# hyperledger-labs/bdls

Hardware: AMD Instinct MI355X
Metric: P-256 ECDSA verifies/sec (fused SHA-256, bit-exact vs Go crypto/ecdsa + Fabric low-S) (higher is better)
Workload: dtype u32; 1 GPU; BASELINE config 2: 1048576 records/GPU, 256B messages, 65536 distinct keys, 1/16 corrupted, fused SHA-256; records_per_gpu=1048576, records_total=1048576, msg_len=256, nkeys=65536, corrupt_den=16, parallelism=shard1 (no collective)

## Files before the change

### bdls_amd/csrc/ec30.h

```cpp
#pragma once
#include "fp30.h"

namespace bh {

struct J30 {
  uint32_t X[9], Y[9], Z[9];
};

BH_HD void j_copy(J30& r, const J30& p) {
  f_copy(r.X, p.X);
  f_copy(r.Y, p.Y);
  f_copy(r.Z, p.Z);
}

BH_HD void j_sel(J30& r, bool c, const J30& a, const J30& b) {
  f_sel(r.X, c, a.X, b.X);
  f_sel(r.Y, c, a.Y, b.Y);
  f_sel(r.Z, c, a.Z, b.Z);
}

template <class F>
BH_HD void j_dbl(J30& r, const J30& p) {
  if constexpr (F::a_is_minus3) {
    uint32_t delta[9], gamma[9], bt[9], t0[9], t1[9], u[9], alpha[9];
    f_sqr<F>(delta, p.Z);
    f_sqr<F>(gamma, p.Y);
    f_mul<F>(bt, p.X, gamma);
    f_sub<F, 32>(t0, p.X, delta);
    f_add(t1, p.X, delta);
    f_mul<F>(u, t0, t1);
    f_mulc<3>(alpha, u);
    f_add(t0, p.Y, p.Z);
    f_sqr<F>(t0, t0);
    f_sub2<F, 32>(r.Z, t0, gamma, delta);
    f_sqr<F>(u, alpha);
    f_mulc<8>(t0, bt);
    f_sub<F, 32>(r.X, u, t0);
    f_mulc<12>(t0, bt);
    f_sub<F, 32>(t0, t0, u);
    f_mul<F>(t0, alpha, t0);
    f_sqr<F>(gamma, gamma);
    f_mulc<8>(gamma, gamma);
    f_sub<F, 32>(r.Y, t0, gamma);
  } else {
    uint32_t A[9], B[9], Cc[9], D[9], E[9], t[9], t2[9];
    f_sqr<F>(A, p.X);
    f_sqr<F>(B, p.Y);
    f_mul<F>(t, p.Y, p.Z);
    f_sqr<F>(Cc, B);
    f_add(t2, p.X, B);
    f_sqr<F>(t2, t2);
    f_mulc<2>(r.Z, t);
    f_add(t, A, Cc);
    f_sub<F, 32>(t2, t2, t);
    f_mulc<2>(D, t2);
    f_mulc<3>(E, A);
    f_sqr<F>(t, E);
    f_mulc<3>(t2, D);
    f_sub<F, 32>(t2, t2, t);
    f_mulc<2>(D, D);
    f_reduce<F>(D, D);
    f_sub<F, 32>(r.X, t, D);
    f_mul<F>(t, E, t2);
    f_mulc<8>(Cc, Cc);
    f_sub<F, 32>(r.Y, t, Cc);
  }
}

template <class F>
BH_HD void j_dblu(J30& r, J30& pp, const J30& p) {
  if constexpr (F::a_is_minus3) {
    uint32_t delta[9], gamma[9], bt[9], t0[9], t1[9], u[9], alpha[9];
    f_sqr<F>(delta, p.Z);
    f_sqr<F>(gamma, p.Y);
    f_mul<F>(bt, p.X, gamma);
    f_sub<F, 32>(t0, p.X, delta);
    f_add(t1, p.X, delta);
    f_mul<F>(u, t0, t1);
    f_mulc<3>(alpha, u);
    f_add(t0, p.Y, p.Z);
    f_sqr<F>(t0, t0);
    f_sub2<F, 32>(r.Z, t0, gamma, delta);
    f_sqr<F>(u, alpha);
    f_mulc<8>(t0, bt);
    f_sub<F, 32>(r.X, u, t0);
    f_mulc<4>(pp.X, bt);
    f_mulc<12>(t0, bt);
    f_sub<F, 32>(t0, t0, u);
    f_mul<F>(t0, alpha, t0);
    f_sqr<F>(gamma, gamma);
    f_mulc<8>(pp.Y, gamma);
    f_sub<F, 32>(r.Y, t0, pp.Y);
    f_copy(pp.Z, r.Z);
  } else {
    uint32_t A[9], B[9], Cc[9], D[9], E[9], t[9], t2[9];
    f_sqr<F>(A, p.X);
    f_sqr<F>(B, p.Y);
    f_mul<F>(t, p.Y, p.Z);
    f_sqr<F>(Cc, B);
    f_add(t2, p.X, B);
    f_sqr<F>(t2, t2);
    f_mulc<2>(r.Z, t);
    f_add(t, A, Cc);
    f_sub<F, 32>(t2, t2, t);
    f_mulc<2>(D, t2);
    f_reduce<F>(D, D);
    f_copy(pp.X, D);
    f_mulc<3>(E, A);
    f_sqr<F>(t, E);
    f_mulc<3>(t2, D);
    f_sub<F, 32>(t2, t2, t);
    f_mulc<2>(D, D);
    f_sub<F, 32>(r.X, t, D);
    f_mul<F>(t, E, t2);
    f_mulc<8>(pp.Y, Cc);
    f_sub<F, 32>(r.Y, t, pp.Y);
    f_copy(pp.Z, r.Z);
  }
}

template <class F>
BH_HD void j_zaddu(J30& r, J30& p, const J30& q) {
  uint32_t t1[9], c[9], w1[9], w2[9], t2[9], d[9], t3[9];
  f_sub<F, 64>(t1, p.X, q.X);
  f_sqr<F>(c, t1);
  f_mul<F>(w1, p.X, c);
  f_mul<F>(w2, q.X, c);
  f_sub<F, 64>(t2, p.Y, q.Y);
  f_sqr<F>(d, t2);
  f_sub<F, 32>(t3, w1, w2);
  f_mul<F>(p.Y, p.Y, t3);
  f_sub2<F, 32>(r.X, d, w1, w2);
  f_sub<F, 64>(t3, w1, r.X);
  f_mul<F>(t3, t2, t3);
  f_sub<F, 32>(r.Y, t3, p.Y);
  f_mul<F>(r.Z, p.Z, t1);
  f_copy(p.X, w1);
  f_copy(p.Z, r.Z);
}

template <class F>
BH_HD bool j_degenerate(const uint32_t z3[9], const uint32_t rr[9], bool* same_y) {
  const bool degenerate = f_is_zero2<F>(z3);
  if (degenerate) {
    uint32_t t[9];
    f_reduce<F>(t, rr);
    uint32_t z = 0;
    for (int i = 0; i < 9; i++) z |= t[i];
    *same_y = (z == 0);
  } else {
    *same_y = false;
  }
  return degenerate;
}

template <class F, bool CO>
BH_HD bool j_add_impl(J30& r, J30* pz, const J30& p, const J30& q, bool neg, bool* same_y) {
  uint32_t z1z1[9], z2z2[9], u1[9], u2[9], s1[9], s2[9], h[9], rr[9], t[9], hh[9], hhh[9], w[9];
  f_sqr<F>(z1z1, p.Z);
  f_sqr<F>(z2z2, q.Z);
  f_mul<F>(u1, p.X, z2z2);
  f_mul<F>(u2, q.X, z1z1);
  f_mul<F>(t, q.Z, z2z2);
  f_mul<F>(s1, p.Y, t);
  f_mul<F>(t, p.Z, z1z1);
  f_mul<F>(s2, q.Y, t);
  f_sub<F, 32>(h, u2, u1);
  f_csub<F, 32>(rr, neg, s2, s1);
  f_sqr<F>(hh, h);
  f_mul<F>(hhh, hh, h);
  f_mul<F>(u1, u1, hh);
  f_sqr<F>(t, rr);
  f_add2x(w, hhh, u1);
  f_sub<F, 32>(r.X, t, w);
  f_addsub<F, 32>(u2, w, u1, t);
  f_mul<F>(u2, rr, u2);
  f_mul<F>(s1, s1, hhh);
  f_sub<F, 32>(r.Y, u2, s1);
  f_mul<F>(t, p.Z, q.Z);
  f_mul<F>(r.Z, t, h);
  if constexpr (CO) {
    f_copy(pz->X, u1);
    f_copy(pz->Y, s1);
    f_copy(pz->Z, r.Z);
  }
  return j_degenerate<F>(r.Z, rr, same_y);
}

template <class F>
BH_HD bool j_add(J30& r, const J30& p, const J30& q, bool* same_y) {
  return j_add_impl<F, false>(r, nullptr, p, q, false, same_y);
}
template <class F>
BH_HD bool j_add_co(J30& r, J30& pz, const J30& p, const J30& q, bool* same_y, bool neg = false) {
  return j_add_impl<F, true>(r, &pz, p, q, neg, same_y);
}

template <class F, bool CO>
BH_HD bool j_madd_impl(J30& r, J30* pz, const J30& p, const uint32_t x2[9], const uint32_t y2[9],
                       bool neg, bool* same_y) {
  uint32_t z1z1[9], u2[9], s2[9], h[9], rr[9], t[9], hh[9], hhh[9], v[9], w[9];
  f_sqr<F>(z1z1, p.Z);
  f_mul<F>(u2, x2, z1z1);
  f_mul<F>(t, p.Z, z1z1);
  f_mul<F>(s2, y2, t);
  f_sub<F, 64>(h, u2, p.X);
  f_csub<F, 96>(rr, neg, s2, p.Y);
  f_sqr<F>(hh, h);
  f_mul<F>(hhh, hh, h);
  f_mul<F>(v, p.X, hh);
  f_sqr<F>(t, rr);
  f_add2x(w, hhh, v);
  f_sub<F, 32>(r.X, t, w);
  f_addsub<F, 32>(s2, w, v, t);
  f_mul<F>(s2, rr, s2);
  f_mul<F>(t, p.Y, hhh);
  f_sub<F, 32>(r.Y, s2, t);
  f_mul<F>(r.Z, p.Z, h);
  if constexpr (CO) {
    f_copy(pz->X, v);
    f_copy(pz->Y, t);
    f_copy(pz->Z, r.Z);
  }
  return j_degenerate<F>(r.Z, rr, same_y);
}

template <class F>
BH_HD bool j_madd(J30& r, const J30& p, const uint32_t x2[9], const uint32_t y2[9], bool* same_y,
                  bool neg = false) {
  return j_madd_impl<F, false>(r, nullptr, p, x2, y2, neg, same_y);
}
template <class F>
BH_HD bool j_madd_co(J30& r, J30& pz, const J30& p, const uint32_t x2[9], const uint32_t y2[9],
                     bool* same_y, bool neg = false) {
  return j_madd_impl<F, true>(r, &pz, p, x2, y2, neg, same_y);
}

template <class F>
BH_HD bool j_on_curve(const uint32_t x[9], const uint32_t y[9]) {
  uint32_t l[9], rhs[9], t[9], b[9];
  f_sqr<F>(l, y);
  f_sqr<F>(t, x);
  f_mul<F>(rhs, t, x);
  if constexpr (F::a_is_minus3) {
    f_mulc<3>(t, x);
    f_sub<F, 32>(rhs, rhs, t);
  }
  f_const(b, F::b_m);
  f_add(rhs, rhs, b);
  f_reduce<F>(rhs, rhs);
  f_canon<F>(l, l);
  return f_eq(l, rhs);
}

}
```

### bdls_amd/csrc/fp30.h

```cpp
#pragma once
#include "bh_common.h"
#include "curve_consts.h"

#ifndef BH_ZFILTER
#define BH_ZFILTER 0
#endif

namespace bh {

constexpr uint32_t kM30 = 0x3fffffffu;
constexpr int kL = 9;

BH_HD void f_copy(uint32_t r[9], const uint32_t a[9]) {
#pragma unroll
  for (int i = 0; i < 9; i++) r[i] = a[i];
}

BH_HD void f_sel(uint32_t r[9], bool c, const uint32_t a[9], const uint32_t b[9]) {
#pragma unroll
  for (int i = 0; i < 9; i++) r[i] = c ? a[i] : b[i];
}

template <class C>
BH_HD void f_const(uint32_t r[9], const C& c) {
#pragma unroll
  for (int i = 0; i < 9; i++) r[i] = c[i];
}

template <uint32_t K>
BH_HD void mac_k(uint64_t& c, uint32_t m) {
#if defined(__HIP_DEVICE_COMPILE__)
  uint32_t k = K;
  asm("" : "+s"(k));
  c += (uint64_t)m * k;
#else
  c += (uint64_t)m * K;
#endif
}

template <class F>
BH_HD void f_redc(uint32_t r[9], uint64_t C[17]) {
  uint64_t acc = 0;
  if constexpr (F::sparse_p256) {
#pragma unroll
    for (int k = 0; k < 8; k++) {
      const uint32_t m = (uint32_t)C[k];
      mac_k<64u>(C[k + 3], m);
      mac_k<4096u>(C[k + 6], m);
      mac_k<F::p[7]>(C[k + 7], m);
      mac_k<F::p[8]>(C[k + 8], m);
      mac_k<4u>(C[k + 1], (uint32_t)(C[k] >> 32));
    }
#pragma unroll
    for (int k = 8; k < 17; k++) {
      acc += C[k];
      const uint32_t m = (uint32_t)acc & kM30;
      if (k == 8) {
        mac_k<64u>(C[11], m);
        mac_k<4096u>(C[14], m);
        mac_k<F::p[7]>(C[15], m);
        mac_k<F::p[8]>(C[16], m);
      } else {
        r[k - 9] = m;
      }
      acc >>= 30;
    }
  } else {
#pragma unroll
    for (int k = 0; k < 17; k++) {
      acc += C[k];
      if (k < 9) {
        const uint32_t m = ((uint32_t)acc * F::n0) & kM30;
        acc += (uint64_t)m * F::p[0];
#pragma unroll
        for (int j = 1; j < 9; j++)
          if (F::p[j]) C[k + j] += (uint64_t)m * F::p[j];
      } else {
        r[k - 9] = (uint32_t)acc & kM30;
      }
      acc >>= 30;
    }
  }
  r[8] = (uint32_t)acc;
}

template <class F>
BH_HD void f_mul(uint32_t r[9], const uint32_t a[9], const uint32_t b[9]) {
  uint64_t C[17];
#pragma unroll
  for (int k = 0; k < 17; k++) C[k] = 0;
#pragma unroll
  for (int i = 0; i < 9; i++)
#pragma unroll
    for (int j = 0; j < 9; j++) C[i + j] += (uint64_t)a[i] * b[j];
  f_redc<F>(r, C);
}

template <class F>
BH_HD void f_sqr(uint32_t r[9], const uint32_t a[9]) {
  uint64_t C[17];
  uint32_t d[9];
#pragma unroll
  for (int i = 0; i < 9; i++) d[i] = a[i] << 1;
#pragma unroll
  for (int k = 0; k < 17; k++) C[k] = 0;
#pragma unroll
  for (int i = 0; i < 9; i++) {
    C[2 * i] += (uint64_t)a[i] * a[i];
#pragma unroll
    for (int j = i + 1; j < 9; j++) C[i + j] += (uint64_t)d[i] * a[j];
  }
  f_redc<F>(r, C);
}

BH_HD void f_add(uint32_t r[9], const uint32_t a[9], const uint32_t b[9]) {
  uint32_t c = 0;
#pragma unroll
  for (int i = 0; i < 8; i++) {
    const uint32_t t = a[i] + b[i] + c;
    r[i] = t & kM30;
    c = t >> 30;
  }
  r[8] = a[8] + b[8] + c;
}

template <class F, int K>
BH_HD void f_sub(uint32_t r[9], const uint32_t a[9], const uint32_t b[9]) {
  static_assert(K == 32 || K == 64, "K");
  uint32_t c = 0;
#pragma unroll
  for (int i = 0; i < 8; i++) {
    const uint32_t kk = (K == 32) ? F::k32[i] : F::k64[i];
    const uint32_t t = a[i] + kk - b[i] + c;
    r[i] = t & kM30;
    c = t >> 30;
  }
  const uint32_t k8 = (K == 32) ? F::k32[8] : F::k64[8];
  r[8] = a[8] + k8 - b[8] + c;
}

struct Limbs9 {
  uint32_t v[9];
};
template <class F, int K, int B>
constexpr Limbs9 kp_borrowed() {
  Limbs9 r{};
  uint64_t c = 0;
  for (int i = 0; i < 9; i++) {
    const uint64_t t = (uint64_t)F::p[i] * (uint64_t)K + c;
    const uint64_t n = i < 8 ? (t & kM30) : t;
    c = i < 8 ? (t >> 30) : 0;
    r.v[i] = (uint32_t)(n + (i < 8 ? ((uint64_t)B << 30) : 0) - (i > 0 ? (uint64_t)B : 0));
  }
  return r;
}
template <class F, int K, int B>
struct KpB {
  static constexpr Limbs9 k = kp_borrowed<F, K, B>();
  static_assert(k.v[8] < (1u << 26), "K p's top limb covers the borrow");
};

BH_HD void f_add2x(uint32_t r[9], const uint32_t a[9], const uint32_t b[9]) {
  uint32_t c = 0;
#pragma unroll
  for (int i = 0; i < 8; i++) {
    const uint32_t t = a[i] + (b[i] << 1) + c;
    r[i] = t & kM30;
    c = t >> 30;
  }
  r[8] = a[8] + (b[8] << 1) + c;
}

template <class F, int K>
BH_HD void f_addsub(uint32_t r[9], const uint32_t a[9], const uint32_t b[9], const uint32_t c[9]) {
  static_assert(K == 32 || K == 64, "K");
  uint32_t cy = 0;
#pragma unroll
  for (int i = 0; i < 8; i++) {
    const uint32_t kk = (K == 32) ? F::k32[i] : F::k64[i];
    const uint32_t t = a[i] + b[i] + kk + cy - c[i];
    r[i] = t & kM30;
    cy = t >> 30;
  }
  const uint32_t k8 = (K == 32) ? F::k32[8] : F::k64[8];
  r[8] = a[8] + b[8] + k8 + cy - c[8];
}

template <class F, int K>
BH_HD void f_sub2(uint32_t r[9], const uint32_t a[9], const uint32_t b[9], const uint32_t c[9]) {
  constexpr Limbs9 kk = KpB<F, K, 2>::k;
  uint32_t cy = 0;
#pragma unroll
  for (int i = 0; i < 8; i++) {
    const uint32_t t = a[i] + kk.v[i] + cy - b[i] - c[i];
    r[i] = t & kM30;
    cy = t >> 30;
  }
  r[8] = a[8] + kk.v[8] + cy - b[8] - c[8];
}

template <class F, int K>
BH_HD void f_csub(uint32_t r[9], bool neg, const uint32_t s[9], const uint32_t y[9]) {
  constexpr Limbs9 kk = KpB<F, K, 2>::k;
  uint32_t cy = 0;
#pragma unroll
  for (int i = 0; i < 8; i++) {
    const uint32_t x = neg ? 0u - s[i] : s[i];
    const uint32_t t = kk.v[i] + x + cy - y[i];
    r[i] = t & kM30;
    cy = t >> 30;
  }
  const uint32_t x8 = neg ? 0u - s[8] : s[8];
  r[8] = kk.v[8] + x8 + cy - y[8];
}

template <class F, int K>
BH_HD void f_neg(uint32_t r[9], const uint32_t a[9]) {
  const uint32_t z[9] = {0, 0, 0, 0, 0, 0, 0, 0, 0};
  f_sub<F, K>(r, z, a);
}

template <uint32_t C>
BH_HD void f_mulc(uint32_t r[9], const uint32_t a[9]) {
  uint64_t c = 0;
#pragma unroll
  for (int i = 0; i < 8; i++) {
    const uint64_t t = (uint64_t)a[i] * C + c;
    r[i] = (uint32_t)t & kM30;
    c = t >> 30;
  }
  r[8] = a[8] * C + (uint32_t)c;
}

template <class F>
BH_HD void f_canon(uint32_t r[9], const uint32_t a[9]) {
  uint32_t d[9];
  int32_t c = 0;
#pragma unroll
  for (int i = 0; i < 8; i++) {
    const int32_t t = (int32_t)a[i] - (int32_t)F::p[i] + c;
    d[i] = (uint32_t)t & kM30;
    c = t >> 30;
  }
  const int32_t t8 = (int32_t)a[8] - (int32_t)F::p[8] + c;
  d[8] = (uint32_t)t8;
  f_sel(r, t8 >= 0, d, a);
}

template <class F>
BH_HD void f_reduce(uint32_t r[9], const uint32_t a[9]) {
  uint32_t one[9];
  f_const(one, F::r1);
  f_mul<F>(r, a, one);
  f_canon<F>(r, r);
}

BH_HD bool f_eq(const uint32_t a[9], const uint32_t b[9]) {
  uint32_t x = 0;
#pragma unroll
  for (int i = 0; i < 9; i++) x |= a[i] ^ b[i];
  return x == 0;
}

template <class F>
BH_HD bool f_is_zero2(const uint32_t a[9]) {
#if BH_ZFILTER
  if (a[0] != 0u && a[0] != F::p[0]) return false;
#endif
  uint32_t z = 0, q = 0;
#pragma unroll
  for (int i = 0; i < 9; i++) {
    z |= a[i];
    q |= a[i] ^ F::p[i];
  }
  return z == 0 || q == 0;
}

BH_HD void f_from_u256(uint32_t r[9], const uint32_t a[8]) {
  r[0] = a[0] & kM30;
#pragma unroll
  for (int i = 1; i < 8; i++) {
    const int lo = 30 * i;
    const int w = lo >> 5, s = lo & 31;
    uint32_t v = a[w] >> s;
    if (s > 2 && w + 1 < 8) v |= a[w + 1] << (32 - s);
    r[i] = v & kM30;
  }
  r[8] = a[7] >> 16;
}

BH_HD void f_to_u256(uint32_t r[8], const uint32_t a[9]) {
#pragma unroll
  for (int w = 0; w < 8; w++) {
    const int bit = 32 * w;
    const int i = bit / 30, s = bit % 30;
    uint32_t v = a[i] >> s;
    if (i + 1 < 9) v |= a[i + 1] << (30 - s);
    if (s > 28 && i + 2 < 9) v |= a[i + 2] << (60 - s);
    r[w] = v;
  }
}

template <class F>
BH_HD void f_to_mont(uint32_t r[9], const uint32_t a[9]) {
  uint32_t r2[9];
  f_const(r2, F::r2);
  f_mul<F>(r, a, r2);
}

template <class F>
BH_HD void f_sqrn(uint32_t r[9], const uint32_t a[9], int k) {
  f_copy(r, a);
#pragma unroll 1
  for (int i = 0; i < k; i++) f_sqr<F>(r, r);
}

template <class F>
BH_HD void f_sqrn_mul(uint32_t r[9], const uint32_t a[9], int k, const uint32_t b[9]) {
  f_sqrn<F>(r, a, k);
  f_mul<F>(r, r, b);
}

template <class F>
BH_HD void f_inv(uint32_t r[9], const uint32_t a[9]) {
  uint32_t e2[9], e3[9], t[9], u[9], acc[9];
  f_sqrn_mul<F>(e2, a, 1, a);
  f_sqrn_mul<F>(e3, e2, 1, a);
  if constexpr (F::sparse_p256) {
    uint32_t e15[9], e32[9];
    f_sqrn_mul<F>(t, e3, 3, e3);
    f_sqrn_mul<F>(u, t, 6, t);
    f_sqrn_mul<F>(e15, u, 3, e3);
    f_sqrn_mul<F>(t, e15, 15, e15);
    f_sqrn_mul<F>(e32, t, 2, e2);
    f_sqrn_mul<F>(acc, e32, 32, a);
    f_sqrn<F>(acc, acc, 96);
    f_sqrn_mul<F>(acc, acc, 32, e32);
    f_sqrn_mul<F>(acc, acc, 32, e32);
    f_sqrn_mul<F>(acc, acc, 30, t);
    f_sqrn_mul<F>(acc, acc, 2, a);
  } else {
    uint32_t e11[9], e22[9], e44[9];
    f_sqrn_mul<F>(t, e3, 3, e3);
    f_sqrn_mul<F>(u, t, 3, e3);
    f_sqrn_mul<F>(e11, u, 2, e2);
    f_sqrn_mul<F>(e22, e11, 11, e11);
    f_sqrn_mul<F>(e44, e22, 22, e22);
    f_sqrn_mul<F>(t, e44, 44, e44);
    f_sqrn_mul<F>(u, t, 88, t);
    f_sqrn_mul<F>(t, u, 44, e44);
    f_sqrn_mul<F>(acc, t, 3, e3);
    f_sqrn_mul<F>(acc, acc, 23, e22);
    f_sqrn_mul<F>(acc, acc, 5, a);
    f_sqrn_mul<F>(acc, acc, 3, e2);
    f_sqrn_mul<F>(acc, acc, 2, a);
  }
  f_copy(r, acc);
}

}
```

### bdls_amd/csrc/verify.h

```cpp
#pragma once
#include <type_traits>

#include "blake2b.h"
#include "der.h"
#include "fe.h"
#include "ec30.h"
#include "sha256.h"
#include "sha3.h"

namespace bh {

enum : uint32_t {
  BHF_HASH_SHA256 = 1u,
  BHF_NO_LOW_S = 2u,
  BHF_HASH_SHA3_256 = 8u,
  BHF_BDLS_PREHASHED = 0x100u,
};

enum : int { HK_GIVEN_OR_SHA256 = 0, HK_SHA3_256 = 1 };

enum : uint8_t { ST_R2OK = 0x80u };

struct BatchIn {
  const uint8_t* pub;
// ... 1223 lines not shown
template <class P, class Raw>
BH_HD void reg_window(uint32_t* tab, uint32_t win, const J30& B, Raw& raw) {
  J30 Bz, S;
  uint32_t z[9];
  raw.store(0u, B);
  f_copy(z, B.Z);
  raw.store_z(0u, z);
  j_dblu<P>(S, Bz, B);
  raw.store(1u, S);
  f_mul<P>(z, z, S.Z);
  raw.store_z(1u, z);
#pragma unroll 1
  for (uint32_t j = 2; j < (uint32_t)kKEnt; j++) {
    J30 T;
    j_zaddu<P>(T, Bz, S);
    raw.store(j, T);
    f_mul<P>(z, z, T.Z);
    raw.store_z(j, z);
    j_copy(S, T);
  }
  uint32_t inv[9];
  f_inv_sg<P>(inv, z);
#pragma unroll 1
  for (uint32_t j = (uint32_t)kKEnt; j-- > 0;) {
    J30 E;
    raw.load(E, j);
    uint32_t zi[9], x[9], y[9];
    if (j > 0) {
      uint32_t pz[9];
      raw.load_z(pz, j - 1u);
      f_mul<P>(zi, inv, pz);
      f_mul<P>(inv, inv, E.Z);
    } else {
      f_copy(zi, inv);
    }
    ll_to_affine<P>(x, y, E, zi);
    llaff_store(tab + kRegWin, win * (uint32_t)kKEnt + j, x, y);
  }
}

struct RegSlotRaw {
  uint32_t* tab;
  BH_HDM void store(uint32_t j, const J30& P) { ktab_store(tab + kRegWinRaw, 0, j, P); }
  BH_HDM void load(J30& P, uint32_t j) const { ktab_load(P, tab + kRegWinRaw, 0, j); }
  BH_HDM void store_z(uint32_t j, const uint32_t z[9]) { z_store(tab + kRegWinPre + 12u * j, z); }
  BH_HDM void load_z(uint32_t z[9], uint32_t j) const { z_load(z, tab + kRegWinPre + 12u * j); }
};

template <class P>
BH_HD void ktab_build_aff(uint32_t* tab, const Work& w, uint32_t rec) {
  J30 B;
  ld9(B.X, w.qx, rec, w.ns);
  ld9(B.Y, w.qy, rec, w.ns);
  f_const(B.Z, P::r1);
  RegSlotRaw raw{tab};
#pragma unroll 1
  for (uint32_t win = 0; win < (uint32_t)kKWin; win++) {
    reg_window<P>(tab, win, B, raw);
    if (win + 1u < (uint32_t)kKWin) {
#pragma unroll 1
      for (int d = 0; d < kKW; d++) j_dbl<P>(B, B);
    }
  }
}

template <class P>
BH_HD void reg_build(uint32_t* tab, const Work& w, uint32_t rec) {
  lltab_build<P>(tab, w, rec);
  ktab_build_aff<P>(tab, w, rec);
}
template <class P>
BH_HD void reg_build_comb(uint32_t* tab, const Work& w, uint32_t rec, uint32_t* scr = nullptr) {
  lltab_build<P>(tab, w, rec, scr);
}

template <class P>
using CvOf = typename std::conditional<P::a_is_minus3 != 0, Cv_p256, Cv_k1>::type;

BH_HD void ll_column(const uint64_t sl[kLLTeeth], int j, uint32_t& idx, bool& neg) {
  uint32_t m = 0;
#pragma unroll
  for (int t = 0; t + 1 < kLLTeeth; t++) m |= (uint32_t)((sl[t] >> j) & 1ull) << t;
  neg = ((sl[kLLTeeth - 1] >> j) & 1ull) == 0ull;
  idx = neg ? (~m & (kLLEnt - 1u)) : m;
}

template <class P>
BH_HD void ll_slices(uint64_t sl[kLLTeeth], const uint32_t u2[8]) {
  using Cv = CvOf<P>;
  const uint32_t add = (u2[0] & 1u) ? 0u : ~0u;
  uint32_t k[9], c[9];
  uint64_t cy = 0;
#pragma unroll
  for (int q = 0; q < 8; q++) {
    cy += (uint64_t)u2[q] + (Cv::n[q] & add);
    k[q] = (uint32_t)cy;
    cy >>= 32;
  }
  k[8] = (uint32_t)cy;
#pragma unroll
  for (int q = 0; q < 8; q++) c[q] = (k[q] >> 1) | (k[q + 1] << 31);
  c[8] = 0u;
  c[(kLLTS - 1) >> 5] |= 1u << ((kLLTS - 1) & 31);
#pragma unroll
  for (int t = 0; t < kLLTeeth; t++) {
    const int lo = kLLSpace * t, wd = lo >> 5, sh = lo & 31;
    uint64_t x = (uint64_t)c[wd] >> sh;
    if (wd + 1 < 9) x |= (uint64_t)c[wd + 1] << (32 - sh);
    if (wd + 2 < 9 && sh + kLLSpace > 64) x |= (uint64_t)c[wd + 2] << (64 - sh);
    sl[t] = x & ((1ull << kLLSpace) - 1ull);
  }
}

template <class P>
BH_HD void q_llcomb(J30& A, bool& a_inf, const Work& w, uint32_t i, const uint32_t* tab,
                    uint32_t stride = 0) {
  uint32_t u2[8], one[9];
  ld8(u2, w.r, i, w.ns);
  f_const(one, P::r1);
  uint64_t sl[kLLTeeth];
  ll_slices<P>(sl, u2);
  uint32_t idx;
  bool neg;
  ll_column(sl, kLLSpace - 1, idx, neg);
  if (stride) llent_load(A.X, A.Y, tab + idx * stride);
  else llaff_load(A.X, A.Y, tab, idx);
  f_copy(A.Z, one);
  a_inf = false;
#pragma unroll 1
  for (int j = kLLSpace - 2; j >= 0; j--) {
    j_dbl<P>(A, A);
    ll_column(sl, j, idx, neg);
    uint32_t tx[9], ty[9], nty[9];
    if (stride) llent_load(tx, ty, tab + idx * stride);
    else llaff_load(tx, ty, tab, idx);
    f_neg<P, 64>(nty, ty);
    f_sel(ty, neg, nty, ty);
    bool same;
    const bool deg = j_madd<P>(A, A, tx, ty, &same);
    if (a_inf || deg) {
      if (a_inf || same) {
        J30 T;
        f_copy(T.X, tx);
        f_copy(T.Y, ty);
        f_copy(T.Z, one);
        if (a_inf) j_copy(A, T);
        else j_dbl<P>(A, T);
        a_inf = false;
      } else {
        a_inf = true;
      }
    }
  }
}

#ifndef BH_GFOLD
#define BH_GFOLD 3
#endif
constexpr int kGF = BH_GFOLD;
static_assert(kGF >= 1 && kGF <= 4 && (kLLSpace - 1) % kGF == 0,
              "column groups of the folded G tables tile columns 1 .. s - 1");
constexpr int kGFBits = (kLLTeeth - 1) + (kGF - 1) * kLLTeeth;
constexpr uint32_t kG2Ent = 1u << kGFBits;
constexpr uint32_t kG1Ent = kLLEnt;
constexpr int kGAdds = (kLLSpace - 1) / kGF + 1;
constexpr uint32_t kGOdd = 1u << (kGF - 1);
constexpr uint32_t kGBase = (uint32_t)kLLTeeth * kGOdd;
constexpr size_t kG2Words = (size_t)(kG2Ent + kG1Ent + kGBase) * kLLAff;
constexpr size_t kGCombWords = (size_t)kCombWindows * kCombEntries * kGEntry;
constexpr size_t kGTabAllWords = kGCombWords + kG2Words;
static_assert(kGCombWords % 4 == 0, "folded tables 16-byte aligned");
BH_HD const uint32_t* g2_of(const uint32_t* gtab) { return gtab + kGCombWords; }

template <class P>
BH_HD void scalar_g_affine(const uint32_t v[9], uint32_t x[9], uint32_t y[9]) {
  uint32_t gx[9], gy[9];
  f_const(gx, P::gx_m);
  f_const(gy, P::gy_m);
  int topbit = 287;
  while (topbit > 0 && !((v[topbit >> 5] >> (topbit & 31)) & 1u)) topbit--;
  J30 A;
  f_copy(A.X, gx);
  f_copy(A.Y, gy);
  f_const(A.Z, P::r1);
  for (int b = topbit - 1; b >= 0; b--) {
    j_dbl<P>(A, A);
    if ((v[b >> 5] >> (b & 31)) & 1u) {
      bool same;
      (void)j_madd<P>(A, A, gx, gy, &same);
    }
  }
  uint32_t z[9], zi[9], zi2[9];
  f_reduce<P>(z, A.Z);
  f_inv<P>(zi, z);
  f_sqr<P>(zi2, zi);
  f_mul<P>(x, A.X, zi2);
  f_mul<P>(zi2, zi2, zi);
  f_mul<P>(y, A.Y, zi2);
  f_reduce<P>(x, x);
  f_reduce<P>(y, y);
}

template <class P>
BH_HD void gtab2_base(uint32_t k, uint32_t* g2) {
  const uint32_t i = k / kGOdd, m = k % kGOdd;
  uint32_t v[9] = {0, 0, 0, 0, 0, 0, 0, 0, 0};
  const int b = kLLSpace * (int)i;
  const uint64_t mag = (uint64_t)(2u * m + 1u) << (b & 31);
  v[b >> 5] = (uint32_t)mag;
  if ((b >> 5) + 1 < 9) v[(b >> 5) + 1] = (uint32_t)(mag >> 32);
  uint32_t x[9], y[9];
  scalar_g_affine<P>(v, x, y);
  llaff_store(g2, kG2Ent + kG1Ent + k, x, y);
}

template <class P>
BH_HD void gtab2_entry(uint32_t t, uint32_t* g2) {
  constexpr uint32_t top = 1u << (kLLTeeth - 1), all = (1u << kLLTeeth) - 1u;
  int c[kLLTeeth];
  for (int i = 0; i < kLLTeeth; i++) c[i] = 0;
  if (t < kG2Ent) {
    for (int cc = 0; cc < kGF; cc++) {
      const uint32_t bits = cc == kGF - 1 ? (top | (t >> ((kGF - 1) * kLLTeeth)))
                                          : (t >> (cc * kLLTeeth)) & all;
      for (int i = 0; i < kLLTeeth; i++) c[i] += (2 * (int)((bits >> i) & 1u) - 1) << cc;
    }
  } else {
    const uint32_t b = top | (t - kG2Ent);
    for (int i = 0; i < kLLTeeth; i++) c[i] = 2 * (int)((b >> i) & 1u) - 1;
  }
  J30 A;
  llaff_load(A.X, A.Y, g2, kG2Ent + kG1Ent + (uint32_t)(kLLTeeth - 1) * kGOdd +
                               (uint32_t)((c[kLLTeeth - 1] - 1) / 2));
  f_const(A.Z, P::r1);
  for (int i = kLLTeeth - 2; i >= 0; i--) {
    const int a = c[i] < 0 ? -c[i] : c[i];
    uint32_t bx[9], by[9];
    llaff_load(bx, by, g2, kG2Ent + kG1Ent + (uint32_t)i * kGOdd + (uint32_t)((a - 1) / 2));
    if (c[i] < 0) f_neg<P, 64>(by, by);
    bool same;
    (void)j_madd<P>(A, A, bx, by, &same);
  }
  uint32_t zi[9], x[9], y[9];
  f_inv_sg<P>(zi, A.Z);
  ll_to_affine<P>(x, y, A, zi);
  llaff_store(g2, t, x, y);
}

BH_HD void g2_column(const uint64_t gl[kLLTeeth], int j, uint32_t& idx, bool& neg) {
  if (j == 0) {
    ll_column(gl, 0, idx, neg);
    idx += kG2Ent;
    return;
  }
  constexpr uint32_t all = (1u << kLLTeeth) - 1u;
  uint32_t col[kGF];
#pragma unroll
  for (int cc = 0; cc < kGF; cc++) {
    uint32_t b = 0;
#pragma unroll
    for (int t = 0; t < kLLTeeth; t++) b |= (uint32_t)((gl[t] >> (j + cc)) & 1ull) << t;
    col[cc] = b;
  }
  neg = ((col[kGF - 1] >> (kLLTeeth - 1)) & 1u) == 0u;
  uint32_t x = col[kGF - 1] & (all >> 1);
  if (neg) x = ~col[kGF - 1] & (all >> 1);
#pragma unroll
  for (int cc = kGF - 2; cc >= 0; cc--) x = (x << kLLTeeth) | ((neg ? ~col[cc] : col[cc]) & all);
  idx = x;
}

template <class P>
BH_HD void ll_madd(J30& A, bool& a_inf, const uint32_t tx[9], uint32_t ty[9], bool neg,
                   const uint32_t one[9]) {
  bool same;
  const bool deg = j_madd<P>(A, A, tx, ty, &same, neg);
  if (a_inf || deg) {
    if (neg) f_neg<P, 64>(ty, ty);
    if (a_inf || same) {
      J30 T;
      f_copy(T.X, tx);
      f_copy(T.Y, ty);
      f_copy(T.Z, one);
      if (a_inf) j_copy(A, T);
      else j_dbl<P>(A, T);
      a_inf = false;
    } else {
      a_inf = true;
    }
  }
}

template <class P>
BH_HD void ll_dbladd(J30& A, bool& a_inf, const uint32_t tx[9], uint32_t ty[9], bool neg,
                     const uint32_t one[9]) {
  if (a_inf) {
    if (neg) f_neg<P, 64>(ty, ty);
    f_copy(A.X, tx);
    f_copy(A.Y, ty);
    f_copy(A.Z, one);
    a_inf = false;
    return;
  }
  J30 R, Az;
  bool same;
  if (j_madd_co<P>(R, Az, A, tx, ty, &same, neg)) {
    if (neg) f_neg<P, 64>(ty, ty);
    J30 T;
    f_copy(T.X, tx);
    f_copy(T.Y, ty);
    f_copy(T.Z, one);
    if (same) {
      j_dbl<P>(A, T);
      (void)j_madd<P>(A, A, tx, ty, &same);
    }
    return;
  }
  j_zaddu<P>(A, R, Az);
  if (f_is_zero2<P>(A.Z)) a_inf = true;
}

template <class P>
BH_HD void q_llcomb_g(J30& A, bool& a_inf, const Work& w, uint32_t i, const uint32_t* tab,
                      uint32_t stride, const uint32_t* g2) {
  uint32_t u2[8], u1[8], one[9];
  ld8(u2, w.r, i, w.ns);
  ld8(u1, w.e, i, w.ns);
  f_const(one, P::r1);
  uint64_t sl[kLLTeeth], gl[kLLTeeth];
  ll_slices<P>(sl, u2);
  ll_slices<P>(gl, u1);
  uint32_t idx;
  bool neg;
  ll_column(sl, kLLSpace - 1, idx, neg);
  if (stride) llent_load(A.X, A.Y, tab + idx * stride);
  else llaff_load(A.X, A.Y, tab, idx);
  f_copy(A.Z, one);
  a_inf = false;
  uint32_t gx[9], gy[9], gidx;
  bool gneg;
  g2_column(gl, kLLSpace - kGF, gidx, gneg);
  llaff_load(gx, gy, g2, gidx);
#pragma unroll 1
  for (int j = kLLSpace - 2; j >= 0; j--) {
    {
      uint32_t tx[9], ty[9];
      ll_column(sl, j, idx, neg);
      if (stride) llent_load(tx, ty, tab + idx * stride);
      else llaff_load(tx, ty, tab, idx);
      ll_dbladd<P>(A, a_inf, tx, ty, neg, one);
    }
    if (j == 0 || (j - 1) % kGF == 0) {
      ll_madd<P>(A, a_inf, gx, gy, gneg, one);
      if (j > 0) {
        g2_column(gl, j > kGF ? j - kGF : 0, gidx, gneg);
        llaff_load(gx, gy, g2, gidx);
      }
    }
  }
}

template <class P>
BH_HD bool stage_keycomb_fold(const Work& w, uint32_t i, const uint32_t* tab, uint32_t stride,
                              const uint32_t* g2) {
  J30 A;
  bool a_inf;
  q_llcomb_g<P>(A, a_inf, w, i, tab, stride, g2);
  return finish_check<P>(w, i, A, a_inf, A, true);
}

#ifndef BH_LADDER_CSUB
#define BH_LADDER_CSUB 1
#endif
template <class P>
BH_HD void j_dbladd(J30& A, bool& a_inf, J30& T, bool neg) {
  if (a_inf) {
    if (neg) f_neg<P, 64>(T.Y, T.Y);
    j_copy(A, T);
    a_inf = false;
    return;
  }
  J30 R, Az;
  bool same;
  if (j_add_co<P>(R, Az, A, T, &same, neg)) {
    if (neg) f_neg<P, 64>(T.Y, T.Y);
    if (same) {
      J30 D;
      j_dbl<P>(D, T);
      (void)j_add<P>(A, D, T, &same);
    }
    return;
  }
  j_zaddu<P>(A, R, Az);
  if (f_is_zero2<P>(A.Z)) a_inf = true;
}

BH_HD bool g_fold_pos(int p) { return p == 0 || (p >= 1 && p <= kLLSpace - kGF && (p - 1) % kGF == 0); }

template <class P>
BH_HD void q_ladder_odd_g(J30& A, bool& a_inf, const Work& w, uint32_t i, uint32_t wave,
                          uint32_t lane, const uint32_t* g2) {
  using Cv = CvOf<P>;
  uint32_t u2[8], u1[8], qx[9], qy[9], one[9];
  ld8(u2, w.r, i, w.ns);
  ld8(u1, w.e, i, w.ns);
  ld9(qx, w.qx, i, w.ns);
  ld9(qy, w.qy, i, w.ns);
  f_const(one, P::r1);
  {
    J30 Qa, D, S;
    f_copy(Qa.X, qx);
    f_copy(Qa.Y, qy);
    f_copy(Qa.Z, one);
    j_dblu<P>(D, S, Qa);
    qtab_store(w.qtab, wave, 0, lane, S);
#pragma unroll 1
    for (uint32_t m = 1; m < (uint32_t)kQTab; m++) {
      J30 Sn;
      j_zaddu<P>(Sn, D, S);
      qtab_store(w.qtab, wave, m, lane, Sn);
      j_copy(S, Sn);
    }
  }
  uint32_t K[9];
  {
    const uint32_t add = (u2[0] & 1u) ? 0u : ~0u;
    uint32_t k[9];
    uint64_t cy = 0;
#pragma unroll
    for (int q = 0; q < 8; q++) {
      cy += (uint64_t)u2[q] + (Cv::n[q] & add);
      k[q] = (uint32_t)cy;
      cy >>= 32;
    }
    k[8] = (uint32_t)cy;
    K[0] = k[0] << 30;
#pragma unroll
    for (int q = 1; q < 9; q++) K[q] = (k[q] << 30) | (k[q - 1] >> 2);
  }
  uint64_t gl[kLLTeeth];
  ll_slices<P>(gl, u1);
  uint32_t gx[9], gy[9], gidx;
  bool gneg;
  int gp = kLLSpace - kGF;
  g2_column(gl, gp, gidx, gneg);
  llaff_load(gx, gy, g2, gidx);
  auto g_add = [&]() {
    ll_madd<P>(A, a_inf, gx, gy, gneg, one);
    if (gp > 0) {
      gp = gp > kGF ? gp - kGF : 0;
      g2_column(gl, gp, gidx, gneg);
      llaff_load(gx, gy, g2, gidx);
    }
  };
  qtab_load(A, w.qtab, wave, (K[8] >> 30) & 1u, lane);
  a_inf = false;
#pragma unroll 1
  for (int win = 50; win >= 0; win--) {
    const uint32_t b = (K[8] >> 25) & 31u;
#pragma unroll
    for (int q = 8; q > 0; q--) K[q] = (K[q] << 5) | (K[q - 1] >> 27);
    K[0] <<= 5;
    const bool neg = b < 16u;
    const uint32_t mag = neg ? 31u - 2u * b : 2u * b - 31u;
    J30 T;
    qtab_load(T, w.qtab, wave, (mag - 1u) >> 1, lane);
#pragma unroll 1
    for (int d = 1; d <= 4; d++) {
      j_dbl<P>(A, A);
      if (g_fold_pos(5 * win + 5 - d)) g_add();
    }
#if BH_LADDER_CSUB
    j_dbladd<P>(A, a_inf, T, neg);
#else
    if (neg) f_neg<P, 64>(T.Y, T.Y);
    j_dbladd<P>(A, a_inf, T, false);
#endif
    if (g_fold_pos(5 * win)) g_add();
  }
}

template <class P>
BH_HD bool stage_ladder_fold(const Work& w, const uint32_t* gtab, uint32_t i, uint32_t wave,
                             uint32_t lane) {
  if constexpr (P::a_is_minus3) {
    J30 A;
    bool a_inf;
    q_ladder_odd_g<P>(A, a_inf, w, i, wave, lane, g2_of(gtab));
    return finish_check<P>(w, i, A, a_inf, A, true);
  } else {
    return stage_ladder<P>(w, gtab, i, wave, lane);
  }
}

template <class P>
BH_HD bool stage_keycomb(const Work& w, const uint32_t* gtab, uint32_t i, const uint32_t* tab,
                         bool aff = false) {
  J30 A, B;
  bool a_inf, b_inf;
  q_keycomb<P>(A, a_inf, w, i, tab, aff);
  uint32_t u1[8];
  ld8(u1, w.e, i, w.ns);
  g_comb<P>(B, b_inf, gtab, u1);
  return finish_check<P>(w, i, A, a_inf, B, b_inf);
}

constexpr uint32_t kGPartWords = 28;
template <class P>
BH_HD void stage_gpart(const Work& w, const uint32_t* gtab, uint32_t i, uint32_t j) {
  J30 B;
  bool b_inf;
  uint32_t u1[8];
  ld8(u1, w.e, i, w.ns);
  g_comb<P>(B, b_inf, gtab, u1);
  uint32_t* o = w.gpart + j;
#pragma unroll
  for (int k = 0; k < 9; k++) {
    o[(size_t)k * w.ns] = B.X[k];
    o[(size_t)(9 + k) * w.ns] = B.Y[k];
    o[(size_t)(18 + k) * w.ns] = B.Z[k];
  }
  o[(size_t)27 * w.ns] = b_inf ? 1u : 0u;
}

template <class P>
BH_HD bool stage_keycomb_q(const Work& w, uint32_t i, uint32_t j, const uint32_t* tab,
                           bool ll = false, uint32_t stride = 0, bool aff = false) {
  J30 A, B;
  bool a_inf;
  if (ll) q_llcomb<P>(A, a_inf, w, i, tab, stride);
  else q_keycomb<P>(A, a_inf, w, i, tab, aff);
  const uint32_t* o = w.gpart + j;
#pragma unroll
  for (int k = 0; k < 9; k++) {
    B.X[k] = o[(size_t)k * w.ns];
    B.Y[k] = o[(size_t)(9 + k) * w.ns];
    B.Z[k] = o[(size_t)(18 + k) * w.ns];
  }
  const bool b_inf = o[(size_t)27 * w.ns] != 0;
  return finish_check<P>(w, i, A, a_inf, B, b_inf);
}

BH_HD uint64_t key_hash(const Work& w, uint32_t i) {
  uint32_t qx[9], qy[9];
  ld9(qx, w.qx, i, w.ns);
  ld9(qy, w.qy, i, w.ns);
  uint64_t h = 0x9e3779b97f4a7c15ull;
#pragma unroll
  for (int k = 0; k < 9; k++) {
    h ^= qx[k];
    h *= 0xff51afd7ed558ccdull;
    h ^= (uint64_t)qy[k] << 32;
    h ^= h >> 29;
  }
  return h ? h : 1;
}

BH_HD bool same_key(const Work& w, uint32_t a, uint32_t b) {
  uint32_t xa[9], ya[9], xb[9], yb[9];
  ld9(xa, w.qx, a, w.ns);
  ld9(ya, w.qy, a, w.ns);
  ld9(xb, w.qx, b, w.ns);
  ld9(yb, w.qy, b, w.ns);
  uint32_t d = 0;
#pragma unroll
  for (int k = 0; k < 9; k++) d |= (xa[k] ^ xb[k]) | (ya[k] ^ yb[k]);
  return d == 0;
}


struct KeyReg {
  uint32_t cap;
  uint32_t hc;
  uint64_t* slot_hash;
  uint32_t* slot_tab;
  uint32_t* keys;
  uint32_t* tables;
  uint32_t* count;
};

constexpr uint32_t kLocal = 0x80000000u;

BH_HD const uint32_t* tab_ptr(const Plan& pl, const KeyReg& g, uint32_t id) {
  return (id & kLocal) ? pl.tables + (size_t)(id & ~kLocal) * kKTabWords
                       : g.tables + (size_t)id * kKTabWords;
}

BH_HD bool reg_key_eq(const KeyReg& g, uint32_t t, const Work& w, uint32_t i) {
  const uint32_t* k = g.keys + (size_t)t * 18;
  uint32_t qx[9], qy[9];
  ld9(qx, w.qx, i, w.ns);
  ld9(qy, w.qy, i, w.ns);
  uint32_t d = 0;
#pragma unroll
  for (int q = 0; q < 9; q++) d |= (k[q] ^ qx[q]) | (k[9 + q] ^ qy[q]);
  return d == 0;
}

BH_HD void reg_key_store(const KeyReg& g, uint32_t t, const Work& w, uint32_t i) {
  uint32_t* k = g.keys + (size_t)t * 18;
  uint32_t qx[9], qy[9];
  ld9(qx, w.qx, i, w.ns);
  ld9(qy, w.qy, i, w.ns);
#pragma unroll
  for (int q = 0; q < 9; q++) {
    k[q] = qx[q];
    k[9 + q] = qy[q];
  }
}

BH_HD uint32_t reg_lookup(const KeyReg& g, const Work& w, uint32_t i, uint64_t h) {
  if (g.cap == 0) return kNone;
  const uint32_t mask = g.hc - 1;
  uint32_t p = (uint32_t)h & mask;
  for (uint32_t probe = 0; probe < g.hc; probe++) {
    const uint64_t cur = g.slot_hash[p];
    if (cur == 0) return kNone;
    if (cur == h) {
      const uint32_t t = g.slot_tab[p];
      if (t < g.cap && reg_key_eq(g, t, w, i)) return t;
    }
    p = (p + 1) & mask;
  }
  return kNone;
}


BH_HD void shr288(uint32_t o[9], const uint32_t v[9], uint32_t sh) {
  const uint32_t ws = sh >> 5, bs = sh & 31u;
  uint32_t t[9];
#pragma unroll
  for (int q = 0; q < 9; q++) {
    uint32_t x = 0;
#pragma unroll
    for (uint32_t d = 0; d < 9; d++)
      if (ws == d) x = (q + (int)d < 9) ? v[q + d] : 0u;
    t[q] = x;
  }
#pragma unroll
  for (int q = 0; q < 9; q++) {
    const uint32_t hi = (q + 1 < 9) ? t[q + 1] : 0u;
    o[q] = bs ? ((t[q] >> bs) | (hi << (32 - bs))) : t[q];
  }
}

template <class P>
BH_HD void j_acc(J30& A, bool& a_inf, const J30& T, bool t_inf) {
  J30 R;
  bool same;
  const bool deg = j_add<P>(R, A, T, &same);
  const bool take = !t_inf;
  const bool use_t = take && a_inf;
  const bool use_r = take && !a_inf && !deg;
  const bool rare = take && !a_inf && deg;
  j_sel(A, use_r, R, A);
  j_sel(A, use_t, T, A);
  if (rare) {
    if (same) j_dbl<P>(A, T);
    else a_inf = true;
  }
  if (use_t) a_inf = false;
}

template <class P>
BH_HD void j_acc_aff(J30& A, bool& a_inf, const uint32_t tx[9], const uint32_t ty[9],
                     const uint32_t one[9], bool t_inf) {
  J30 R;
  bool same;
  const bool deg = j_madd<P>(R, A, tx, ty, &same);
  const bool take = !t_inf;
  const bool use_t = take && a_inf;
  const bool use_r = take && !a_inf && !deg;
  const bool rare = take && !a_inf && deg;
  j_sel(A, use_r, R, A);
  if (use_t) {
    f_copy(A.X, tx);
    f_copy(A.Y, ty);
    f_copy(A.Z, one);
  }
  if (rare) {
    if (same) {
      J30 T;
      f_copy(T.X, tx);
      f_copy(T.Y, ty);
      f_copy(T.Z, one);
      j_dbl<P>(A, T);
    } else {
      a_inf = true;
    }
  }
  if (use_t) a_inf = false;
}

template <class P, int L>
BH_HD void g_comb_part(J30& C, bool& c_inf, const uint32_t* gtab, const uint32_t u1[8],
                       uint32_t l);
// ... 97 lines not shown
```

Measured before the change: 192.0 million verifies/s.

## Fuse add+co-Z add into double-add with lazy products and dual-product reduction

Replaces the co-Z add followed by a separate zaddu with a single fused double-and-add routine, j_zaddc. It reuses the difference values (x1-x3 and 2·y1-s) directly, which saves the t1 subtraction and several copies. It also adds f_mul2, which computes a·b + c·d with one shared P-256 sparse reduction, and uses it in the Y coordinate of the plain add, madd and zaddc. This is meant to cut reductions and register traffic in the ladder's hot loop, at the risk of wider 64-bit column accumulators that depend on the proved column bound, plus higher register pressure.

After: 196.3 million verifies/s, median of 6. 2.2% higher.

```diff
diff --git a/bdls_amd/csrc/ec30.h b/bdls_amd/csrc/ec30.h
--- a/bdls_amd/csrc/ec30.h
+++ b/bdls_amd/csrc/ec30.h
@@ -154,8 +154,31 @@
   return degenerate;
 }
 
-template <class F, bool CO>
-BH_HD bool j_add_impl(J30& r, J30* pz, const J30& p, const J30& q, bool neg, bool* same_y) {
+template <class F, bool FUSE = true>
+BH_HD void j_zaddc(J30& r, const uint32_t x1[9], const uint32_t y1[9], const uint32_t x2[9],
+                   const uint32_t dx[9], const uint32_t sy[9], const uint32_t z[9]) {
+  uint32_t c[9], w1[9], w2[9], t2[9], d[9], t3[9], t4[9];
+  f_sqr<F>(c, dx);
+  f_mul<F>(w1, x1, c);
+  f_mul<F>(w2, x2, c);
+  f_dblsub<F, 32>(t2, y1, sy);
+  f_sqr<F>(d, t2);
+  f_sub2<F, 32>(r.X, d, w1, w2);
+  f_sub<F, 64>(t3, w1, r.X);
+  if constexpr (F::sparse_p256 && FUSE) {
+    f_sub<F, 32>(t4, w2, w1);
+    f_mul2<F>(r.Y, t2, t3, y1, t4);
+  } else {
+    f_sub<F, 32>(t4, w1, w2);
+    f_mul<F>(t4, y1, t4);
+    f_mul<F>(t3, t2, t3);
+    f_sub<F, 32>(r.Y, t3, t4);
+  }
+  f_mul<F>(r.Z, z, dx);
+}
+
+template <class F, bool DA>
+BH_HD bool j_add_impl(J30& r, const J30& p, const J30& q, bool neg, bool* same_y) {
   uint32_t z1z1[9], z2z2[9], u1[9], u2[9], s1[9], s2[9], h[9], rr[9], t[9], hh[9], hhh[9], w[9];
   f_sqr<F>(z1z1, p.Z);
   f_sqr<F>(z2z2, q.Z);
@@ -172,33 +195,46 @@
   f_mul<F>(u1, u1, hh);
   f_sqr<F>(t, rr);
   f_add2x(w, hhh, u1);
-  f_sub<F, 32>(r.X, t, w);
-  f_addsub<F, 32>(u2, w, u1, t);
-  f_mul<F>(u2, rr, u2);
-  f_mul<F>(s1, s1, hhh);
-  f_sub<F, 32>(r.Y, u2, s1);
-  f_mul<F>(t, p.Z, q.Z);
-  f_mul<F>(r.Z, t, h);
-  if constexpr (CO) {
-    f_copy(pz->X, u1);
-    f_copy(pz->Y, s1);
-    f_copy(pz->Z, r.Z);
-  }
-  return j_degenerate<F>(r.Z, rr, same_y);
+  if constexpr (DA) {
+    uint32_t x3[9], z3[9];
+    f_sub<F, 32>(x3, t, w);
+    f_addsub<F, 32>(u2, w, u1, t);
+    f_mul<F>(s2, rr, u2);
+    f_mul<F>(s1, s1, hhh);
+    f_mul<F>(t, p.Z, q.Z);
+    f_mul<F>(z3, t, h);
+    if (j_degenerate<F>(z3, rr, same_y)) return true;
+    j_zaddc<F, false>(r, u1, s1, x3, u2, s2, z3);
+    return false;
+  } else {
+    f_sub<F, 32>(r.X, t, w);
+    f_addsub<F, 32>(u2, w, u1, t);
+    if constexpr (F::sparse_p256) {
+      f_neg<F, 32>(s2, s1);
+      f_mul2<F>(r.Y, rr, u2, s2, hhh);
+    } else {
+      f_mul<F>(u2, rr, u2);
+      f_mul<F>(s1, s1, hhh);
+      f_sub<F, 32>(r.Y, u2, s1);
+    }
+    f_mul<F>(t, p.Z, q.Z);
+    f_mul<F>(r.Z, t, h);
+    return j_degenerate<F>(r.Z, rr, same_y);
+  }
 }
 
 template <class F>
 BH_HD bool j_add(J30& r, const J30& p, const J30& q, bool* same_y) {
-  return j_add_impl<F, false>(r, nullptr, p, q, false, same_y);
-}
-template <class F>
-BH_HD bool j_add_co(J30& r, J30& pz, const J30& p, const J30& q, bool* same_y, bool neg = false) {
-  return j_add_impl<F, true>(r, &pz, p, q, neg, same_y);
-}
-
-template <class F, bool CO>
-BH_HD bool j_madd_impl(J30& r, J30* pz, const J30& p, const uint32_t x2[9], const uint32_t y2[9],
-                       bool neg, bool* same_y) {
+  return j_add_impl<F, false>(r, p, q, false, same_y);
+}
+template <class F>
+BH_HD bool j_add_da(J30& r, const J30& p, const J30& q, bool* same_y, bool neg = false) {
+  return j_add_impl<F, true>(r, p, q, neg, same_y);
+}
+
+template <class F, bool DA>
+BH_HD bool j_madd_impl(J30& r, const J30& p, const uint32_t x2[9], const uint32_t y2[9], bool neg,
+                       bool* same_y) {
   uint32_t z1z1[9], u2[9], s2[9], h[9], rr[9], t[9], hh[9], hhh[9], v[9], w[9];
   f_sqr<F>(z1z1, p.Z);
   f_mul<F>(u2, x2, z1z1);
@@ -211,29 +247,41 @@
   f_mul<F>(v, p.X, hh);
   f_sqr<F>(t, rr);
   f_add2x(w, hhh, v);
-  f_sub<F, 32>(r.X, t, w);
-  f_addsub<F, 32>(s2, w, v, t);
-  f_mul<F>(s2, rr, s2);
-  f_mul<F>(t, p.Y, hhh);
-  f_sub<F, 32>(r.Y, s2, t);
-  f_mul<F>(r.Z, p.Z, h);
-  if constexpr (CO) {
-    f_copy(pz->X, v);
-    f_copy(pz->Y, t);
-    f_copy(pz->Z, r.Z);
-  }
-  return j_degenerate<F>(r.Z, rr, same_y);
+  if constexpr (DA) {
+    uint32_t x3[9], z3[9];
+    f_sub<F, 32>(x3, t, w);
+    f_addsub<F, 32>(u2, w, v, t);
+    f_mul<F>(s2, rr, u2);
+    f_mul<F>(t, p.Y, hhh);
+    f_mul<F>(z3, p.Z, h);
+    if (j_degenerate<F>(z3, rr, same_y)) return true;
+    j_zaddc<F>(r, v, t, x3, u2, s2, z3);
+    return false;
+  } else {
+    f_sub<F, 32>(r.X, t, w);
+    f_addsub<F, 32>(s2, w, v, t);
+    if constexpr (F::sparse_p256) {
+      f_negk<F, 96>(u2, p.Y);
+      f_mul2<F>(r.Y, rr, s2, u2, hhh);
+    } else {
+      f_mul<F>(s2, rr, s2);
+      f_mul<F>(t, p.Y, hhh);
+      f_sub<F, 32>(r.Y, s2, t);
+    }
+    f_mul<F>(r.Z, p.Z, h);
+    return j_degenerate<F>(r.Z, rr, same_y);
+  }
 }
 
 template <class F>
 BH_HD bool j_madd(J30& r, const J30& p, const uint32_t x2[9], const uint32_t y2[9], bool* same_y,
                   bool neg = false) {
-  return j_madd_impl<F, false>(r, nullptr, p, x2, y2, neg, same_y);
-}
-template <class F>
-BH_HD bool j_madd_co(J30& r, J30& pz, const J30& p, const uint32_t x2[9], const uint32_t y2[9],
+  return j_madd_impl<F, false>(r, p, x2, y2, neg, same_y);
+}
+template <class F>
+BH_HD bool j_madd_da(J30& r, const J30& p, const uint32_t x2[9], const uint32_t y2[9],
                      bool* same_y, bool neg = false) {
-  return j_madd_impl<F, true>(r, &pz, p, x2, y2, neg, same_y);
+  return j_madd_impl<F, true>(r, p, x2, y2, neg, same_y);
 }
 
 template <class F>
diff --git a/bdls_amd/csrc/fp30.h b/bdls_amd/csrc/fp30.h
--- a/bdls_amd/csrc/fp30.h
+++ b/bdls_amd/csrc/fp30.h
@@ -124,6 +124,32 @@
   r[8] = a[8] + b[8] + c;
 }
 
+template <class F>
+BH_HD void f_mul2(uint32_t r[9], const uint32_t a[9], const uint32_t b[9], const uint32_t c[9],
+                  const uint32_t d[9]) {
+  static_assert(F::sparse_p256, "f_mul2: the column bound is proved for the sparse P-256 f_redc only");
+  uint64_t C[17];
+#pragma unroll
+  for (int k = 0; k < 17; k++) C[k] = 0;
+#pragma unroll
+  for (int i = 0; i < 9; i++)
+#pragma unroll
+    for (int j = 0; j < 9; j++) C[i + j] += (uint64_t)a[i] * b[j];
+  uint32_t hi[9];
+#pragma unroll
+  for (int k = 4; k <= 12; k++) {
+    hi[k - 4] = (uint32_t)(C[k] >> 32);
+    C[k] = (uint32_t)C[k];
+  }
+#pragma unroll
+  for (int k = 4; k <= 12; k++) mac_k<4u>(C[k + 1], hi[k - 4]);
+#pragma unroll
+  for (int i = 0; i < 9; i++)
+#pragma unroll
+    for (int j = 0; j < 9; j++) C[i + j] += (uint64_t)c[i] * d[j];
+  f_redc<F>(r, C);
+}
+
 template <class F, int K>
 BH_HD void f_sub(uint32_t r[9], const uint32_t a[9], const uint32_t b[9]) {
   static_assert(K == 32 || K == 64, "K");
@@ -212,6 +238,34 @@
   }
   const uint32_t x8 = neg ? 0u - s[8] : s[8];
   r[8] = kk.v[8] + x8 + cy - y[8];
+}
+
+template <class F, int K>
+BH_HD void f_negk(uint32_t r[9], const uint32_t a[9]) {
+  constexpr Limbs9 kk = KpB<F, K, 1>::k;
+  uint32_t cy = 0;
+#pragma unroll
+  for (int i = 0; i < 8; i++) {
+    const uint32_t t = kk.v[i] + cy - a[i];
+    r[i] = t & kM30;
+    cy = t >> 30;
+  }
+  r[8] = kk.v[8] + cy - a[8];
+}
+
+template <class F, int K>
+BH_HD void f_dblsub(uint32_t r[9], const uint32_t a[9], const uint32_t b[9]) {
+  static_assert(K == 32 || K == 64, "K");
+  uint32_t cy = 0;
+#pragma unroll
+  for (int i = 0; i < 8; i++) {
+    const uint32_t kk = (K == 32) ? F::k32[i] : F::k64[i];
+    const uint32_t t = (a[i] << 1) + kk + cy - b[i];
+    r[i] = t & kM30;
+    cy = t >> 30;
+  }
+  const uint32_t k8 = (K == 32) ? F::k32[8] : F::k64[8];
+  r[8] = (a[8] << 1) + k8 + cy - b[8];
 }
 
 template <class F, int K>
diff --git a/bdls_amd/csrc/verify.h b/bdls_amd/csrc/verify.h
--- a/bdls_amd/csrc/verify.h
+++ b/bdls_amd/csrc/verify.h
@@ -1549,9 +1549,8 @@
     a_inf = false;
     return;
   }
-  J30 R, Az;
   bool same;
-  if (j_madd_co<P>(R, Az, A, tx, ty, &same, neg)) {
+  if (j_madd_da<P>(A, A, tx, ty, &same, neg)) {
     if (neg) f_neg<P, 64>(ty, ty);
     J30 T;
     f_copy(T.X, tx);
@@ -1563,7 +1562,6 @@
     }
     return;
   }
-  j_zaddu<P>(A, R, Az);
   if (f_is_zero2<P>(A.Z)) a_inf = true;
 }
 
@@ -1627,9 +1625,8 @@
     a_inf = false;
     return;
   }
-  J30 R, Az;
   bool same;
-  if (j_add_co<P>(R, Az, A, T, &same, neg)) {
+  if (j_add_da<P>(A, A, T, &same, neg)) {
     if (neg) f_neg<P, 64>(T.Y, T.Y);
     if (same) {
       J30 D;
@@ -1638,7 +1635,6 @@
     }
     return;
   }
-  j_zaddu<P>(A, R, Az);
   if (f_is_zero2<P>(A.Z)) a_inf = true;
 }
 
```
